# liruihan000/game_engine

Hardware: AMD Instinct MI355X
Metric: room-phase steps/sec (higher is better)
Workload: dtype u32

## Files before the change

game_engine_amd/csrc/ge_device.h:

```cpp
#pragma once
#include <hip/hip_runtime.h>
#include "ge_layout.h"

namespace ge {

enum { COMP_UI = 0, COMP_TIMER = 1, COMP_ACTION = 2 };
enum { ACT_NONE = 0, ACT_WOLF_TARGET, ACT_DOCTOR_PROTECT, ACT_DETECTIVE, ACT_DAY_VOTE,
       ACT_TT_STATEMENTS, ACT_TT_LIE, ACT_TT_VOTE };
enum { EFF_NONE = 0, EFF_ASSIGN_ROLES, EFF_NIGHT_BEGIN, EFF_NIGHT_RESOLVE, EFF_DAY_RESOLVE,
       EFF_TT_ROUND_START, EFF_TT_REVEAL, EFF_TT_SCORE };
enum { RES_ALWAYS = 0, RES_WOLVES_ZERO, RES_WOLVES_GE_VILLAGERS, RES_FOLLOWS_DAY, RES_FOLLOWS_NIGHT,
       RES_ALL_ROUNDS_DONE, RES_OTHERWISE };

constexpr uint32_t GOLDEN = 0x9E3779B9u;

#ifndef GE_SINGLE_GLOBAL
#define GE_SINGLE_GLOBAL 5
#endif
template <bool LOWOCC, bool SINGLE> constexpr bool single_global(int game_bit) { return SINGLE && ((GE_SINGLE_GLOBAL >> (game_bit + (LOWOCC ? 0 : 1))) & 1) != 0; }
#ifndef GE_DEAL_EARLY
#define GE_DEAL_EARLY 1
#endif
#ifndef GE_STAMPS
#define GE_STAMPS 0
#endif
#ifndef GE_RES_PACKED
#define GE_RES_PACKED 1
#endif
#ifndef GE_QUEUE_PRIO
#define GE_QUEUE_PRIO 3
#endif
#ifndef GE_RES_ATOMIC64
#define GE_RES_ATOMIC64 1
#endif
#ifndef GE_RESOLVE_PRIO
#define GE_RESOLVE_PRIO 2
#endif
#ifndef GE_TALLY_BYTES
#define GE_TALLY_BYTES 1
#endif
#ifndef GE_COLD_FALLBACK
#define GE_COLD_FALLBACK 1
#endif
#ifndef GE_COLD_DEAL_NOW
#define GE_COLD_DEAL_NOW 0
#endif
#ifndef GE_LONE_DEAL_WORDS
#define GE_LONE_DEAL_WORDS 1
#endif
#ifndef GE_TAIL_KNOWN_RESTART
#define GE_TAIL_KNOWN_RESTART 1
#endif
#ifndef GE_ROW_DERIVED
#define GE_ROW_DERIVED 1
#endif
#ifndef GE_CTX_PERM
#define GE_CTX_PERM 0
#endif
#ifndef GE_SKIP_MASK
#define GE_SKIP_MASK 0
#endif
#ifndef GE_RES_UNMASKED
#define GE_RES_UNMASKED 0
#endif
#ifndef GE_ROWS_SPLIT
#define GE_ROWS_SPLIT 1
#endif
#ifndef GE_DEAL_PERIOD
#define GE_DEAL_PERIOD 16
#endif

template <int NB, bool LOWOCC, bool SINGLE = false> struct WwBuild {
    static constexpr bool ORD = NB <= 8;
    static constexpr bool ONE_ATOMIC = NB <= 8 && LOWOCC;
    static constexpr bool SHADOW = LOWOCC || NB <= 8;
    static constexpr bool ONEHOT = LOWOCC && NB <= 8;
    static constexpr bool PIN_CHOICE = LOWOCC && NB > 8;
    static constexpr bool SEL_OPEN = LOWOCC;
    static constexpr bool TPL_TRACE = LOWOCC;
    static constexpr int DEAL_FORM = SINGLE ? 2 : NB <= 8 ? ((LOWOCC && !GE_LONE_DEAL_WORDS) ? 0 : 1) : LOWOCC ? 0 : 2;
    static constexpr bool DEAL_EARLY = GE_DEAL_EARLY && !LOWOCC && !SINGLE;
    static constexpr bool TABLE = !LOWOCC;
    static constexpr bool LONE = LOWOCC && NB <= 8 && !SINGLE;
};

GE_HD uint32_t mix32(uint32_t x) {
    x ^= x >> 16; x *= 0x7FEB352Du; x ^= x >> 15; x *= 0x846CA68Bu; x ^= x >> 16;
    return x;
}
GE_HD uint32_t room_key(uint32_t seed_lo, uint32_t seed_hi, uint64_t room) {
    uint32_t k = mix32(seed_lo ^ 0x243F6A88u);
    k = mix32(k ^ seed_hi);
    k = mix32(k ^ (uint32_t)room);
    k = mix32(k ^ (uint32_t)(room >> 32));
    return k;
}
GE_HD uint32_t seed_key(uint32_t seed_lo, uint32_t seed_hi) { return mix32(mix32(seed_lo ^ 0x243F6A88u) ^ seed_hi); }
GE_HD uint32_t room_key_from(uint32_t sk, uint64_t room) { return mix32(mix32(sk ^ (uint32_t)room) ^ (uint32_t)(room >> 32)); }
GE_HD uint32_t turn_key(uint32_t rk, uint32_t turn) { return mix32(rk ^ (turn * GOLDEN)); }
GE_HD uint32_t draw(uint32_t tk, uint32_t idx) { return mix32(tk + (idx + 1u) * GOLDEN); }
GE_HD uint32_t deal_key(uint32_t rk, uint32_t game) { return mix32(rk ^ 0x44454C31u ^ (game * GOLDEN)); }

#if defined(__HIPCC__)
__device__ __forceinline__ uint32_t pick(uint32_t d, uint32_t k) { return __umulhi(d, k); }
__device__ __forceinline__ uint32_t popc(uint32_t x) { return (uint32_t)__popc(x); }
__device__ __forceinline__ uint32_t ctz(uint32_t x) { return (uint32_t)__ffs((int)x) - 1u; }

template <int NB> __device__ __forceinline__ uint32_t nth_set_bit(uint32_t m, uint32_t n) {
    uint32_t pos = 0, c;
    if (NB > 8) { c = popc(m & 0xFFu); if (n >= c) { n -= c; pos = 8; m >>= 8; } }
    c = popc(m & 0xFu); if (n >= c) { n -= c; pos += 4; m >>= 4; }
    c = popc(m & 0x3u); if (n >= c) { n -= c; pos += 2; m >>= 2; }
    c = m & 1u;         if (n >= c) { pos += 1; }
    return pos;
}

__device__ __forceinline__ uint32_t nth_set_bit_swar8(uint32_t m, uint32_t n) {
    uint32_t x = m & 0xFFu;
    x = (x | (x << 12)) & 0x000F000Fu; x = (x | (x << 6)) & 0x03030303u; x = (x | (x << 3)) & 0x11111111u;
    const uint32_t t = (x + 7u - n) * 0x11111111u;
    return (uint32_t)__builtin_ctz((t & 0x88888888u) | 0x80000000u) >> 2;
}

template <int NB> __device__ __forceinline__ uint32_t nth_set_bit_lds(const uint8_t *nth8, uint32_t m, uint32_t n) {
    if (NB <= 8) return nth8[(m & 0xFFu) * 8u + (n & 7u)];
    const uint32_t lo = m & 0xFFu, c = popc(lo);
    const bool in_lo = n < c;
    const uint32_t idx = in_lo ? lo * 8u + n : ((m >> 8) & 0xFFu) * 8u + ((n - c) & 7u);
    return (in_lo ? 0u : 8u) + nth8[idx];
}

inline void fill_nth8_host(uint8_t *nth8) {
    for (uint32_t m = 0; m < 256u; m++) {
        uint32_t x = m;
        for (uint32_t n = 0; n < 8u; n++) {
            uint32_t pos = 0;
            while (x && !((x >> pos) & 1u)) pos++;
            nth8[m * 8u + n] = (uint8_t)(x ? pos : 0u);
            x &= x - 1u;
        }
    }
}

inline void fill_vote_luts_host(uint32_t *spread8, uint64_t *tally64) {
    for (uint32_t m = 0; m < 256u; m++) {
        uint32_t v = 0;
// ... 35 lines not shown
        const uint2 *tally64 = reinterpret_cast<const uint2 *>(static_cast<const unsigned char *>(img) + IMG_TALLY);
        uint32_t v_lo = (uint32_t)votes & spread8[voters & 0xFFu], v_hi = 0;
        if (NB > 8) v_hi = (uint32_t)((uint64_t)votes >> 32) & spread8[(voters >> 8) & 0xFFu];
        uint32_t lo = 0, hi = 0;
#pragma unroll
        for (int k = 0; k < 4; k++) { const uint2 t = tally64[(v_lo >> (8 * k)) & 0xFFu]; lo += t.x; hi += t.y; }
        if (NB > 8) {
#pragma unroll
            for (int k = 0; k < 2; k++) { const uint2 t = tally64[(v_hi >> (8 * k)) & 0xFFu]; lo += t.x; hi += t.y; }
        }
        const uint32_t a = (lo & 0x00F000F0u) | 0x000A000Eu;
        const uint32_t b = ((lo >> 4) & 0x00F000F0u) | 0x0009000Du;
        const uint32_t c = ((lo >> 8) & 0x00F000F0u) | 0x0008000Cu;
        const uint32_t d = ((lo >> 12) & 0x000000F0u) | ((hi & 15u) << 20) | 0x0007000Bu;
        u16x2 m = __builtin_elementwise_max(__builtin_elementwise_max(pk(a), pk(b)), __builtin_elementwise_max(pk(c), pk(d)));
        if (NB > 8) {
            const uint32_t e = (hi & 0x000000F0u) | ((hi << 12) & 0x00F00000u) | 0x00050006u;
            const uint32_t f = ((hi >> 8) & 0x000000F0u) | ((hi << 4) & 0x00F00000u) | 0x00030004u;
            m = __builtin_elementwise_max(m, __builtin_elementwise_max(pk(e), pk(f)));
        }
        const uint32_t key = m.x > m.y ? m.x : m.y;
        return (key >> 4) ? 15u - (key & 15u) : 0u;
    }
    nib_t vm;
    if (NB <= 8) {
        uint32_t x = voters & 0xFFu;
        x = (x | (x << 12)) & 0x000F000Fu; x = (x | (x << 6)) & 0x03030303u; x = (x | (x << 3)) & 0x11111111u;
        vm = (nib_t)nib_fill(x);
    } else {
        uint64_t x = voters & 0xFFFFu;
        x = (x | (x << 24)) & 0x000000FF000000FFull; x = (x | (x << 12)) & 0x000F000F000F000Full;
        x = (x | (x << 6)) & 0x0303030303030303ull; x = (x | (x << 3)) & 0x1111111111111111ull;
        vm = (nib_t)nib_fill(x);
    }
    const nib_t v = votes & vm;
    uint32_t key = 0;
    if (NB <= 8) {
        const uint32_t v32 = (uint32_t)v;
        uint32_t tally = 0;
        if (GE_TALLY_BYTES) {
            const uint32_t ev = (v32 << 2) & 0x3C3C3C3Cu, od = (v32 >> 2) & 0x3C3C3C3Cu, one = 1u;
            tally = (shl_by_byte<0>(one, ev) + shl_by_byte<0>(one, od) + shl_by_byte<1>(one, ev)) + (shl_by_byte<1>(one, od) + shl_by_byte<2>(one, ev))
                  + (shl_by_byte<2>(one, od) + shl_by_byte<3>(one, ev)) + shl_by_byte<3>(one, od);
        } else {
#pragma unroll
            for (int i = 0; i < NB; i++) tally += 1u << ((4u * ((v32 >> (4 * i)) & 15u)) & 31u);
        }
        {
            const uint32_t c8 = popc(v32 & 0x88888888u);
            const uint32_t a = (tally & 0x00F000F0u) | 0x000A000Eu;
            const uint32_t b = ((tally >> 4) & 0x00F000F0u) | 0x0009000Du;
            const uint32_t c = ((tally >> 8) & 0x00F000F0u) | 0x0008000Cu;
            const uint32_t d = ((tally >> 12) & 0x000000F0u) | (c8 << 20) | 0x0007000Bu;
            const u16x2 m = __builtin_elementwise_max(__builtin_elementwise_max(pk(a), pk(b)), __builtin_elementwise_max(pk(c), pk(d)));
            key = m.x > m.y ? m.x : m.y;
        }
    } else {
        uint64_t tally = 0;
#pragma unroll
        for (int i = 0; i < NB; i++) tally += uint64_t(1) << (4u * ((uint32_t)(v >> (4 * i)) & 15u));
        const uint32_t lo = (uint32_t)tally, hi = (uint32_t)(tally >> 32);
        const uint32_t a = (lo & 0x00F000F0u) | 0x000A000Eu;
        const uint32_t b = ((lo >> 4) & 0x00F000F0u) | 0x0009000Du;
        const uint32_t c = ((lo >> 8) & 0x00F000F0u) | 0x0008000Cu;
        const uint32_t d = ((lo >> 12) & 0x000000F0u) | ((hi & 15u) << 20) | 0x0007000Bu;
        const uint32_t e = (hi & 0x000000F0u) | ((hi << 12) & 0x00F00000u) | 0x00050006u;
        const uint32_t f = ((hi >> 8) & 0x000000F0u) | ((hi << 4) & 0x00F00000u) | 0x00030004u;
        const u16x2 m = __builtin_elementwise_max(__builtin_elementwise_max(__builtin_elementwise_max(pk(a), pk(b)), __builtin_elementwise_max(pk(c), pk(d))),
                                                  __builtin_elementwise_max(pk(e), pk(f)));
        key = m.x > m.y ? m.x : m.y;
    }
    return (key >> 4) ? 15u - (key & 15u) : 0u;
}

struct WaveLds {
    uint4 ctx[64];
    uint4 res[64];
    uint8_t queue[64 * 13];
};
struct WaveLdsLow {
    uint4 slot[64 * 13 + 80];
    uint4 res[64];
};
template <bool LOWOCC> struct WaveLdsOf { using type = WaveLds; };
template <> struct WaveLdsOf<true> { using type = WaveLdsLow; };

template <bool SPLIT>
__device__ __forceinline__ DevRow lds_row(const DevRow *rows, uint32_t idx) {
    if (!(SPLIT && GE_ROWS_SPLIT)) return rows[idx];
    const uint4 *h = reinterpret_cast<const uint4 *>(rows);
    const uint4 a = h[idx], b = h[GE_MAX_PHASES + idx];
    return DevRow{a.x, a.y, a.z, a.w, b.x, b.y, b.z, b.w};
}

__device__ __forceinline__ void wave_sync() {
    __builtin_amdgcn_fence(__ATOMIC_RELEASE, "wavefront");
    __builtin_amdgcn_wave_barrier();
    __builtin_amdgcn_fence(__ATOMIC_ACQUIRE, "wavefront");
}

__device__ __forceinline__ void wave_excl_scan(uint32_t cnt, uint32_t &off, uint32_t &total) {
    uint32_t v = cnt;
    v += (uint32_t)__builtin_amdgcn_update_dpp(0, (int)v, 0x111, 0xf, 0xf, false);
    v += (uint32_t)__builtin_amdgcn_update_dpp(0, (int)v, 0x112, 0xf, 0xf, false);
    v += (uint32_t)__builtin_amdgcn_update_dpp(0, (int)v, 0x114, 0xf, 0xf, false);
    v += (uint32_t)__builtin_amdgcn_update_dpp(0, (int)v, 0x118, 0xf, 0xf, false);
    v += (uint32_t)__builtin_amdgcn_update_dpp(0, (int)v, 0x142, 0xa, 0xf, false);
    v += (uint32_t)__builtin_amdgcn_update_dpp(0, (int)v, 0x143, 0xc, 0xf, false);
    off = v - cnt;
    total = (uint32_t)__builtin_amdgcn_readlane((int)v, 63);
}

struct Stamps {
    unsigned long long last, acc[4];
    __device__ __forceinline__ void start() { last = __builtin_amdgcn_s_memtime(); acc[0] = acc[1] = acc[2] = acc[3] = 0; }
    __device__ __forceinline__ void mark(int k) { const unsigned long long now = __builtin_amdgcn_s_memtime(); acc[k] += now - last; last = now; }
    unsigned long long m0, r0;
    __device__ __forceinline__ void clocks_start() { m0 = __builtin_amdgcn_s_memtime(); r0 = __builtin_amdgcn_s_memrealtime(); }
};

__device__ __forceinline__ uint32_t sel32(bool c, uint32_t a, uint32_t b) { return b ^ ((a ^ b) & (0u - (uint32_t)c)); }

template <int NB, bool TABLE>
__device__ __forceinline__ uint32_t ww_choose(uint32_t act, uint32_t i, uint32_t d, uint32_t alive, uint32_t team_w,
                                              uint32_t known, uint32_t lo_kw, uint32_t r_det, const uint8_t *nth8) {
    const uint32_t me = 1u << i;
    const uint32_t others = alive & ~me, non_wolf = alive & ~team_w;
    const uint32_t fresh = others & ~known;
    uint32_t cand;
    if (!TABLE) {
        const uint32_t det_c = sel32(fresh != 0u, fresh, others);
        const uint32_t vote = sel32((team_w & me) != 0u, non_wolf, sel32((r_det & me) != 0u && lo_kw != 0u, lo_kw, others));
        cand = alive;
        cand = sel32(act == ACT_WOLF_TARGET, non_wolf, cand);
        cand = sel32(act == ACT_DETECTIVE, det_c, cand);
        cand = sel32(act == ACT_DAY_VOTE, vote, cand);
        cand = sel32(cand != 0u, cand, alive);
    } else {
        cand = alive;
        cand = act == ACT_WOLF_TARGET ? non_wolf : cand;
        cand = act == ACT_DETECTIVE ? (fresh ? fresh : others) : cand;
        const uint32_t vote = (team_w & me) ? non_wolf : (((r_det & me) && lo_kw) ? lo_kw : others);
        cand = act == ACT_DAY_VOTE ? vote : cand;
        cand = cand ? cand : alive;
    }
    const uint32_t idx = pick(d, popc(cand));
    return (TABLE ? nth_set_bit_lds<NB>(nth8, cand, idx) : NB <= 8 ? nth_set_bit_swar8(cand, idx) : nth_set_bit<NB>(cand, idx)) + 1u;
}

__device__ __forceinline__ uint32_t bit_mask(uint32_t x, uint32_t pos) {
    uint32_t m = (uint32_t)__builtin_amdgcn_sbfe((int)x, pos, 1u);
    asm("" : "+v"(m));
    return m;
}
__device__ __forceinline__ uint32_t bfi(uint32_t m, uint32_t a, uint32_t b) { return (m & a) | (~m & b); }
__device__ __forceinline__ uint32_t bfi_uniform(uint32_t m, uint32_t a, uint32_t b) {
    uint32_t r;
    asm("v_bfi_b32 %0, %1, %2, %3" : "=v"(r) : "v"(m), "s"(a), "v"(b));
    return r;
}

__device__ __forceinline__ uint32_t ww_choose_onehot8(uint32_t x, uint32_t i, uint32_t d, uint32_t known, uint32_t lo_kw, uint32_t det_voter) {
    const uint32_t alive = x & 0xFFFFu, team_w = (x >> 16) & 0xFFFu;
    const uint32_t me = 1u << i;
    const uint32_t others = alive & ~me, non_wolf = alive & ~team_w;
    const uint32_t fresh = others & ~known;
// ... 309 lines not shown
    uint32_t n, nw, phase0_idx, rkey;
    uint32_t human;
    uint32_t term_mask;
};

enum { TAIL_NONE = 0, TAIL_RUNTIME = 1, TAIL_RECYCLE = 2, TAIL_KEEP = 3 };
template <int NB> struct WwRestart {
    const WWR<NB> *s0;
    uint32_t term_rs;
    uint32_t restarted;
    uint32_t q;
};

template <int NB, bool LOWOCC, int GENERIC, bool DER = false>
__device__ __forceinline__ uint32_t ww_targets(const WWR<NB> &s, const DevRow &row, const WwCtx &c, uint32_t alive, uint32_t ALL) {
    using R = WWR<NB>;
    const uint32_t comp = row.r0 & 3u, nterms = (row.r0 >> 8) & 7u;
    uint32_t T = 0;
    const bool generic_row = GENERIC && (row.r0 & ROW_GENERIC);
    if (LOWOCC ? !GENERIC || !generic_row : (comp == COMP_ACTION && !generic_row)) {
        uint32_t X;
        if (NB <= 8) {
            X = __builtin_amdgcn_perm(s.W[1], s.W[0], row.r4) & __builtin_amdgcn_perm(s.W[2], s.W[2], row.r5);
            X ^= row.r7;
            X &= X >> 16; X &= X >> 8;
        } else {
            X = __builtin_amdgcn_perm(s.W[1], s.W[0], row.r4) & __builtin_amdgcn_perm(s.W[R::NW > 3 ? 3 : 0], s.W[2], row.r5) &
                __builtin_amdgcn_perm(s.W[R::NW - 1], s.W[R::NW - 2], row.r6);
            X ^= row.r7;
            X &= X >> 16;
            if (nterms > 2u) {
                auto term = [&](uint32_t j) -> uint32_t {
                    const uint32_t e = (row.r1 >> (8u * j)) & 255u;
                    const uint32_t wi = e >> 5;
                    uint32_t word = 0xFFFFFFFFu;
#pragma unroll
                    for (int k = 0; k < R::NW; k++) word = wi == (uint32_t)k ? s.W[k] : word;
                    const uint32_t m = word >> (e & 31u);
                    return m ^ (uint32_t)((int32_t)(row.r0 << (15u - j)) >> 31);
                };
                X &= term(2) & term(3);
            }
        }
        T = DER ? X & alive & row.r6 : X & alive & (comp == COMP_ACTION ? ALL : 0u);
    }
    if (generic_row && comp == COMP_ACTION)
        T = ww_cond_generic<NB>(s, c.cc, row.r0, ALL) & alive;
    return T;
}

struct WwBranch {
    bool open;
    uint32_t qe;
};
template <int NB>
__device__ __forceinline__ void ww_phase_branch(const WWR<NB> &s, const DevRow &row, uint32_t phase0_idx, uint32_t alive, uint32_t team_w, WwBranch &b) {
    const bool guard = s.phase == phase0_idx && !(s.flags & FLAG_PHASE0_DONE);
    b.open = !guard;
    const uint32_t w = popc(alive & team_w), g = popc(alive & s.template get<F_TEAM_V>());
    static_assert(EFF_DAY_RESOLVE == 4 && RES_FOLLOWS_DAY == 3 && EFF_NIGHT_RESOLVE == 3 && RES_FOLLOWS_NIGHT == 4 && FLAG_PHASE0_DONE == 1,
                  "the constant below is made for these codes");
    const uint32_t follows = (0xC00u >> (s.flags & 0xEu)) & 0x18u;
    const uint32_t C = 1u | ((w == 0u) << RES_WOLVES_ZERO) | ((w >= g) << RES_WOLVES_GE_VILLAGERS) | follows | (1u << RES_OTHERWISE);
    const uint32_t hit = row.r2 & __builtin_amdgcn_perm(C, C, 0u);
    const uint32_t sh = ctz(hit) & 24u;
    b.qe = hit != 0u ? ((row.r3 >> sh) & 255u) : s.phase;
}

template <int NB, bool LOWOCC, bool SINGLE, bool COLD = false>
__device__ __forceinline__ void ww_prepare_deal(const WWR<NB> &s, const WwCtx &c, Deal &deal, bool deal_now, uint32_t ALL, WWR<NB> &dealt) {
    using B = WwBuild<NB, LOWOCC, SINGLE>;
    const uint32_t g = deal_next_game<NB>(s);
    if ((COLD ? __builtin_expect(deal_now, false) : deal_now) && deal.gv != (g | DEAL_VALID)) {
        deal_roles<NB, B::TABLE, B::DEAL_FORM>(deal, deal_key(c.rkey, g), g, c.n, c.nw, c.nth8);
    }
    if (B::DEAL_FORM != DEAL_PACKED) deal_words<NB, B::DEAL_FORM>(deal, ALL, dealt);
}

struct WwActs { uint32_t newly, det_v, det_w; };

template <int NB, bool LOWOCC, bool FUSED = false, bool LONE8 = false, bool SKIP_GIVEN = false, typename S1, typename S2>
__device__ __forceinline__ void ww_queue_actions(WWR<NB> &s, const WwCtx &c, uint32_t T, uint32_t act, bool night, uint32_t alive, uint32_t team_w,
                                                 uint32_t r_det, uint32_t tk, WwActs &out, S1 &&shadow1, S2 &&shadow2, Stamps *stamps,
                                                 uint32_t rowd = 0u, uint32_t nmask = 0u, uint32_t skip = 0u) {
    using nib_t = typename WWR<NB>::nib_t;
    using B = WwBuild<NB, LOWOCC>;
    constexpr bool DER = LONE8 && GE_ROW_DERIVED, PERM = LONE8 && GE_CTX_PERM && NB <= 8, UNMASKED = LONE8 && GE_RES_UNMASKED && B::ONE_ATOMIC;
    constexpr bool SKIPM = GE_SKIP_MASK && SKIP_GIVEN;
    auto *lw = static_cast<typename WaveLdsOf<LOWOCC>::type *>(c.wave_lds);
    const uint32_t todo = SKIPM ? (T & ~s.acted & ~skip) : c.valid ? (T & ~s.acted & ~c.human) : 0u;
    const uint32_t known = s.det_v | s.det_w;
    const uint32_t kw_alive = s.det_w & alive;
    const uint32_t lo_kw = kw_alive & (0u - kw_alive);
    const uint32_t lane = __lane_id();
    const uint32_t cnt = popc(todo);
#if GE_QUEUE_PRIO
    if (!LOWOCC) __builtin_amdgcn_s_setprio(GE_QUEUE_PRIO);
#endif
    uint32_t ord = 0;
    if (B::ORD) ord = c.ord8[todo & 0xFFu];
    uint32_t off, total;
    wave_excl_scan(cnt, off, total);
    out.newly = 0; out.det_v = 0; out.det_w = 0;
    if (!(LOWOCC || total != 0u)) {
#if GE_QUEUE_PRIO
        __builtin_amdgcn_s_setprio(0);
#endif
        shadow1();
        shadow2();
        return;
    }
    const uint32_t ky = DER ? bfi(nmask, known, lo_kw != 0u ? r_det : 0u) : night ? known : (B::ONEHOT ? (lo_kw != 0u ? r_det : 0u) : r_det);
    const uint32_t kind = B::ONEHOT ? ((1u << act) >> 1) : act;
    static_assert(F_ALIVE == 0 && F_TEAM_W == 7, "the selector below is made for this layout");
    const uint32_t at = PERM ? __builtin_amdgcn_perm(s.W[1], s.W[0], 0x0C070C00u) : alive | (team_w << 16);
    const uint32_t x0 = DER ? at | (rowd & (0xFu << ROWD_KIND_SHIFT)) : at | (kind << 28);
    const uint4 ctx = B::ORD ? make_uint4(x0, ky | (lo_kw << 8) | (off << 16) | (lane << 26), ord, tk)
                             : make_uint4(alive | (team_w << 16) | (act << 28), ky | (lo_kw << 16), todo | (off << 16) | (lane << 26), tk);
    constexpr uint32_t RW = (NB <= 8 && GE_RES_PACKED) ? 2u : 4u;
    uint32_t *const res_w = reinterpret_cast<uint32_t *>(lw->res);
    if (NB <= 8) *reinterpret_cast<uint2 *>(res_w + RW * lane) = make_uint2(0u, 0u);
    else lw->res[lane] = make_uint4(0u, 0u, 0u, 0u);
    if (LOWOCC) {
        auto *lo = reinterpret_cast<WaveLdsLow *>(lw);
        uint4 *qp = lo->slot + (cnt != 0u ? off : 64u * 13u + lane);
#pragma unroll
        for (int j = NB - 1; j >= 0; j--) {
            qp[j] = ctx;
            asm volatile("" ::: "memory");
        }
    } else {
        auto *hi = reinterpret_cast<WaveLds *>(lw);
        hi->ctx[lane] = ctx;
        if (cnt != 0u) {
            uint8_t *qp = hi->queue + off;
#pragma unroll
            for (int j = NB - 1; j >= 0; j--) {
                qp[j] = (uint8_t)lane;
                asm volatile("" ::: "memory");
            }
        }
    }
    wave_sync();
    auto fetch = [&](uint32_t k) -> uint4 {
        if (LOWOCC) return reinterpret_cast<WaveLdsLow *>(lw)->slot[k];
        auto *hi = reinterpret_cast<WaveLds *>(lw);
        return hi->ctx[hi->queue[k] & 63u];
    };
    uint4 c4 = fetch(lane);
    if (B::SHADOW) shadow1();
    constexpr bool PEEL = LOWOCC && FUSED && B::SHADOW;
    if (PEEL) {
        auto round = [&](uint32_t base, auto first_c) {
            const uint32_t k = base + lane;
            if (GE_STAMPS == 1 && stamps && base == 0u) { asm volatile("" :: "v"(c4.x)); stamps->mark(1); }
            uint32_t L, i, know, lokw;
            if (B::ORD) {
                L = c4.y >> 26;
                const uint32_t rank = (k - ((c4.y >> 16) & 0x3FFu)) & 7u;
                i = (c4.z >> (4u * rank)) & 7u;
                know = c4.y & 0xFFu; lokw = (c4.y >> 8) & 0xFFu;
            } else {
                L = c4.z >> 26;
                const uint32_t due = c4.z & 0xFFFFu, rank = (k - ((c4.z >> 16) & 0x3FFu)) & 15u;
                i = nth_set_bit<NB>(due | (1u << 31), rank) & 15u;
                know = c4.y & 0xFFFFu; lokw = c4.y >> 16;
            }
            const uint32_t d = draw(c4.w, i);
            const bool go = k < total && (d & 3u) != 0u;
            uint32_t ch = B::ONEHOT ? ww_choose_onehot8(c4.x, i, d, know, lokw, know)
                                    : ww_choose<NB, false>(c4.x >> 28, i, d, c4.x & 0xFFFFu, (c4.x >> 16) & 0xFFFu, know, lokw, know, c.nth8);
            if (B::PIN_CHOICE) asm volatile("" : "+v"(ch));
            if (UNMASKED && decltype(first_c)::value) {
                atomicOr(res_w + RW * L + 1, go ? ch << (4u * i) : 0u);
            } else if (go) {
                uint32_t *r = res_w + RW * L;
                if (!B::ONE_ATOMIC) atomicOr(r, 1u << i);
                atomicOr(r + 1 + (i >> 3), ch << (4u * (i & 7u)));
            }
        };
        shadow2();
        round(0u, std::true_type{});
        for (uint32_t base = 64u; base < total; base += 64u) {
            c4 = fetch(base + lane);
            round(base, std::false_type{});
        }
    } else {
        for (uint32_t base = 0;; base += 64u) {
            const uint32_t k = base + lane;
            if (GE_STAMPS == 1 && stamps && base == 0u) { asm volatile("" :: "v"(c4.x)); stamps->mark(1); }
            uint32_t L, i, know, lokw;
            if (B::ORD) {
                L = c4.y >> 26;
                const uint32_t rank = (k - ((c4.y >> 16) & 0x3FFu)) & 7u;
                i = (c4.z >> (4u * rank)) & 7u;
                know = c4.y & 0xFFu; lokw = (c4.y >> 8) & 0xFFu;
            } else {
                L = c4.z >> 26;
                const uint32_t due = c4.z & 0xFFFFu, rank = (k - ((c4.z >> 16) & 0x3FFu)) & 15u;
                i = (LOWOCC ? nth_set_bit<NB>(due | (1u << 31), rank) : nth_set_bit_lds<NB>(c.nth8, due, rank)) & 15u;
                know = c4.y & 0xFFFFu; lokw = c4.y >> 16;
            }
            const uint32_t d = draw(c4.w, i);
            const bool go = k < total && (d & 3u) != 0u;
            if (LOWOCC) {
                uint32_t ch = B::ONEHOT ? ww_choose_onehot8(c4.x, i, d, know, lokw, know)
                                        : ww_choose<NB, false>(c4.x >> 28, i, d, c4.x & 0xFFFFu, (c4.x >> 16) & 0xFFFu, know, lokw, know, c.nth8);
                if (B::PIN_CHOICE) asm volatile("" : "+v"(ch));
                if (go) {
                    uint32_t *r = res_w + RW * L;
                    if (!B::ONE_ATOMIC) atomicOr(r, 1u << i);
                    atomicOr(r + 1 + (i >> 3), ch << (4u * (i & 7u)));
                }
            } else if (go) {
                const uint32_t ch = ww_choose<NB, true>(c4.x >> 28, i, d, c4.x & 0xFFFFu, (c4.x >> 16) & 0xFFFu, know, lokw, know, c.nth8);
                uint32_t *r = res_w + RW * L;
                if (NB <= 8 && GE_RES_PACKED && GE_RES_ATOMIC64) {
                    atomicOr(reinterpret_cast<unsigned long long *>(r), (unsigned long long)(1u << i) | ((unsigned long long)(ch << (4u * i)) << 32));
                } else {
                    atomicOr(r, 1u << i);
                    atomicOr(r + 1 + (i >> 3), ch << (4u * (i & 7u)));
                }
            }
            if (base + 64u >= total) break;
            c4 = fetch(k + 64u);
        }
    }
    wave_sync();
    const uint4 r = NB <= 8 ? make_uint4(reinterpret_cast<const uint2 *>(res_w + RW * lane)->x, reinterpret_cast<const uint2 *>(res_w + RW * lane)->y, 0u, 0u)
                            : lw->res[lane];
    if (B::SHADOW) {
        if (!PEEL) shadow2();
// ... 92 lines not shown
        if (B::DEAL_FORM == DEAL_PACKED) deal_words<NB, B::DEAL_FORM>(deal, ALL, dealt);
#pragma unroll
        for (int k = 0; k < R::NW; k++) s.W[k] = (s.W[k] & ~dmask.W[k]) | dealt.W[k];
        deal.gv = 0u;
    } else if (eff == EFF_NIGHT_RESOLVE || eff == EFF_DAY_RESOLVE) {
#if GE_RESOLVE_PRIO
        __builtin_amdgcn_s_setprio(GE_RESOLVE_PRIO);
#endif
        resolve(true, eff == EFF_DAY_RESOLVE);
#if GE_RESOLVE_PRIO
        __builtin_amdgcn_s_setprio(0);
#endif
    }
    const bool nbeg = eff == EFF_NIGHT_BEGIN;
    s.template clear<F_SUB>(nbeg ? R::FM : 0u);
    s.sel = nbeg ? nib_t(0) : s.sel;
    if (!TAILR) {
        s.acted = 0; s.choice = 0;
        s.flags = (s.flags & FLAG_PHASE0_DONE) | (p_eff << 1);
        s.prev = s.phase;
        s.phase = q;
        const bool terminal = SINGLE ? ((c.term_mask >> q) & 1u) != 0u : ((qrow.r0 >> 11) & 7u) == 0u;
        s.end_turn = (terminal && s.end_turn == END_NONE) ? (turn < 0xFFFEu ? turn : 0xFFFEu) : s.end_turn;
    } else {
        s.acted &= ~moved; s.choice &= (nib_t)~moved;
        s.flags = bfi(moved, GE_ROW_DERIVED ? (row.r6 >> ROWD_FLAGS_SHIFT) & 0xFFu : (s.flags & FLAG_PHASE0_DONE) | (p_eff << 1), s.flags);
        s.prev = bfi(moved, s.phase, s.prev);
        s.phase = q;
        if (TAILR != TAIL_RECYCLE) {
            const bool terminal = ((qrow.r0 >> 11) & 7u) == 0u;
            s.end_turn = (terminal && moved != 0u && s.end_turn == END_NONE) ? (turn < 0xFFFEu ? turn : 0xFFFEu) : s.end_turn;
        }
    }
    if (TAILR == TAIL_RUNTIME || TAILR == TAIL_RECYCLE) {
#pragma unroll
        for (int k = 0; k < R::NW; k++) s.W[k] = bfi_uniform(rmask, s0->W[k], s.W[k]);
        s.acted |= rmask & s0->acted; s.choice |= (nib_t)rmask & s0->choice;
        s.det_v = bfi_uniform(rmask, s0->det_v, s.det_v); s.det_w = bfi_uniform(rmask, s0->det_w, s.det_w);
        s.sel = (nib_t)bfi_uniform(rmask, (uint32_t)s0->sel, (uint32_t)s.sel);
        s.phase = bfi_uniform(rmask, s0->phase, s.phase); s.prev = bfi_uniform(rmask, s0->prev, s.prev);
        s.flags = bfi_uniform(rmask, s0->flags, s.flags); s.end_turn = bfi_uniform(rmask, s0->end_turn, s.end_turn);
        const uint32_t g = s.games - rmask;
        s.games = g < 0xFFFFu ? g : 0xFFFFu;
    }
}

template <int NB, bool LOWOCC, int GENERIC = false, bool SINGLE = false, int TAILR = TAIL_NONE>
__device__ __forceinline__ void ww_turn(WWR<NB> &s, DevRow &row, const WwCtx &c, uint32_t turn, uint32_t &tk_io, bool trace, Deal &deal, bool deal_now,
                                        uint32_t &ev_newly, uint64_t &ev_choice, Stamps *stamps = nullptr, WwRestart<NB> *rst = nullptr, uint32_t skip = 0u) {
    static_assert(!TAILR || (NB <= 8 && LOWOCC && !SINGLE), "tail recycling is the fused lone-wavefront Werewolf x 8 form");
    using R = WWR<NB>;
    using B = WwBuild<NB, LOWOCC, SINGLE>;
    const uint32_t ALL = (1u << c.n) - 1u;
    const uint32_t comp = row.r0 & 3u, act = (row.r0 >> 2) & 7u;
    const uint32_t alive = s.template get<F_ALIVE>(), team_w = s.template get<F_TEAM_W>(), r_det = s.template get<F_DET>();
    const bool night = act >= ACT_WOLF_TARGET && act <= ACT_DETECTIVE;

    constexpr bool LONE8 = B::LONE && GENERIC == 0, DER = LONE8 && GE_ROW_DERIVED;
    const uint32_t rowd = row.r6, nmask = DER ? bit_mask(rowd, ROWD_NIGHT_BIT) : 0u;

    const uint32_t T = ww_targets<NB, LOWOCC, GENERIC, DER>(s, row, c, alive, ALL);
    if (GE_STAMPS == 1 && stamps) { asm volatile("" :: "v"(T)); stamps->mark(0); }

    WwBranch br;
    R dealt;
    if (B::DEAL_EARLY) ww_prepare_deal<NB, LOWOCC, SINGLE>(s, c, deal, deal_now, ALL, dealt);
    uint32_t tk_next = 0;
    WwActs acts;
    ww_queue_actions<NB, LOWOCC, !SINGLE, LONE8, TAILR == TAIL_RECYCLE || TAILR == TAIL_KEEP>(s, c, T, act, night, alive, team_w, r_det, tk_io, acts,
        [&]() {
            ww_phase_branch<NB>(s, row, c.phase0_idx, alive, team_w, br);
            if (B::SHADOW) asm volatile("" : "+v"(br.qe));
        },
        [&]() {
            if (!SINGLE) tk_next = turn_key(c.rkey, turn + 1u);
            if (!B::DEAL_EARLY) ww_prepare_deal<NB, LOWOCC, SINGLE, TAILR != TAIL_NONE && GE_COLD_DEAL_NOW>(s, c, deal, deal_now, ALL, dealt);
            if (B::SHADOW) {
                if (!SINGLE) asm volatile("" : "+v"(tk_next));
                if (B::DEAL_FORM != DEAL_PACKED && !B::DEAL_EARLY && !(LOWOCC && B::DEAL_FORM == DEAL_WORDS)) {
#pragma unroll
                    for (int k = 0; k < R::NW; k++) asm volatile("" : "+v"(dealt.W[k]));
                }
            }
        }, stamps, rowd, nmask, skip);
    s.acted |= acts.newly;
    s.template set<F_SUB>(DER ? acts.newly & nmask : night ? acts.newly : 0u);
    ev_newly = acts.newly;
    if (trace) {
        uint64_t m = 0;
#pragma unroll
        for (int i = 0; i < NB; i++) m |= (uint64_t)((acts.newly >> i) & 1u) << (4 * i);
        ev_choice = (uint64_t)s.choice & nib_fill(m);
    }

    tk_io = tk_next;
    s.flags |= FLAG_PHASE0_DONE;
    const uint32_t qe = ww_decide<NB, LOWOCC, DER>(s, comp, T, br);
    {
        const uint32_t seen = acts.det_v | acts.det_w;
        s.det_v = (s.det_v & ~seen) | acts.det_v;
        s.det_w = (s.det_w & ~seen) | acts.det_w;
    }
    if (SINGLE) {
        if ((qe & 31u) != s.phase) ww_apply_effect<NB, LOWOCC, true>(s, row, row, c, qe, alive, ALL, turn, deal, dealt);
    } else if (TAILR) {
        const uint32_t q = qe & 31u;
        const uint32_t moved = 0u - (uint32_t)(q != s.phase);
        const uint32_t rmask = TAILR == TAIL_KEEP ? 0u : bit_mask(rst->term_rs, q);
        const DevRow qrow = lds_row<false>(c.rows, TAILR == TAIL_KEEP ? q : bfi_uniform(rmask, c.phase0_idx, q));
        ww_apply_effect<NB, LOWOCC, false, TAILR>(s, row, qrow, c, qe, alive, ALL, turn, deal, dealt, rmask, rst->s0, moved);
        row = qrow;
        rst->q = q;
        rst->restarted = rmask & 1u;
    } else if ((qe & 31u) != s.phase) {
        const DevRow qrow = lds_row<!LOWOCC>(c.rows, qe & 31u);
        ww_apply_effect<NB, LOWOCC, false>(s, row, qrow, c, qe, alive, ALL, turn, deal, dealt);
        row = qrow;
    }
}

template <int NB> __device__ __forceinline__ uint32_t tt_done_mask(uint64_t rounds_nib, uint32_t R) {
    uint32_t m = 0;
#pragma unroll
    for (int i = 0; i < NB; i++) m |= (((uint32_t)(rounds_nib >> (4 * i)) & 15u) >= R ? 1u : 0u) << i;
    return m;
}

template <int NB, bool QUEUE, bool TABLE, int GENERIC = false, bool SINGLE = false>
__device__ __forceinline__ void tt_turn(TT<NB> &s, uint32_t &done, DevRow &row, const DevRow *rows, const CondCtx &cc, void *wave_lds, const uint8_t *nth8,
                                        bool valid, uint32_t n, uint32_t rounds,
                                        uint32_t phase0_idx, uint32_t rkey, uint32_t turn,
                                        bool trace, uint32_t human, uint32_t term_mask, uint32_t &ev_newly, uint64_t &ev_choice) {
    const uint32_t ALL = (1u << n) - 1u;
    const uint32_t comp = row.r0 & 3u, act = (row.r0 >> 2) & 7u, p_eff = (row.r0 >> 5) & 7u;
    const uint32_t nterms = (row.r0 >> 8) & 7u;
    const uint32_t tk = turn_key(rkey, turn);

    uint32_t T = 0;
    const bool generic_row = GENERIC && (row.r0 & ROW_GENERIC);
    if (comp == COMP_ACTION && !generic_row) {
        const uint32_t W0 = s.speaker | (s.submitted << 16), W1 = s.revealed | (s.can_vote << 16), W2 = s.has_voted;
        uint32_t X = __builtin_amdgcn_perm(W1, W0, row.r4) & __builtin_amdgcn_perm(W2, W2, row.r5);
        X ^= row.r7;
        X &= X >> 16;
        if (nterms > 2u) {
            auto term = [&](uint32_t j) -> uint32_t {
                const uint32_t e = (row.r1 >> (8u * j)) & 255u;
                const uint32_t wi = e >> 5;
                uint32_t word = 0xFFFFFFFFu;
                word = wi == 0u ? W0 : word; word = wi == 1u ? W1 : word; word = wi == 2u ? W2 : word;
                const uint32_t m = word >> (e & 31u);
                return m ^ (uint32_t)((int32_t)(row.r0 << (15u - j)) >> 31);
            };
            X &= term(2) & term(3);
        }
        T = X & ALL;
    }
    if (generic_row && comp == COMP_ACTION)
        T = tt_cond_generic<NB, GENERIC>(s, cc, row.r0, ALL);

    uint32_t newly = 0;
    {
        uint32_t todo = valid ? (T & ~s.acted & ~human) : 0u;
        const bool a_stm = act == ACT_TT_STATEMENTS, a_lie = act == ACT_TT_LIE, a_vote = act == ACT_TT_VOTE;
        if (!QUEUE) {
            while (todo) {
                const uint32_t i = ctz(todo);
// ... 127 lines not shown
```

game_engine_amd/csrc/ge_step.hip:

```cpp
#include <hip/hip_runtime.h>
#include <stdint.h>
#include <stdio.h>
#include <stdlib.h>
#include <string.h>
#include <sched.h>
#include <algorithm>
#include <atomic>
#include <new>
#include <string>
#include <thread>
#include <type_traits>
#include <vector>

#include "../../include/ge_step.h"
#include "ge_device.h"
#include "ge_layout.h"
#include "ge_host.h"

using namespace ge;

namespace {

#include "ge_kernels.inl"

// ... 240 lines not shown
                s.dev.base = reinterpret_cast<uint32_t *>(static_cast<char *>(b->state) + reinterpret_cast<size_t>(s.dev.base));
                DevTable &dt = host_tables[k];
                memset(&dt, 0, sizeof dt);
                for (int r = 0; r < s.table.n_phases; r++) {
                    dt.rows[r] = to_dev_row(s.table, s.table.rows[r], s.dev.kind, s.dev.n_players);
                    dt.conds[r] = to_dev_cond(s.table.rows[r]);
                    if (s.table.rows[r].generic) b->generic = true;
                }
                build_cond_image(s.table, s.dev.kind, dt);
                b->cond_bytes = std::max<uint32_t>(b->cond_bytes, dt.cond_n16 * 16u);
                if (b->segs.size() == 1 && s.table.pack == GE_PACK_TWO_TRUTHS && dt.cond_n16) {
                    static const bool no_shapes = getenv("GE_NO_GENERIC_SHAPES") != nullptr;
                    const uint32_t ncl = dt.cond_shape & 7u, len = (dt.cond_shape >> 4) & 7u;
                    b->gshape = no_shapes ? 0u : (ncl == 1u && len == 1u) ? 2u : (ncl == 1u && len == 2u) ? 3u : 0u;
                }
                dt.n_phases = s.table.n_phases; dt.rounds = s.table.rounds; dt.n_players = (int32_t)s.dev.n_players;
                fill_nth8_host(dt.nth8);
                fill_ord8_host(dt.ord8);
                fill_vote_luts_host(dt.spread8, dt.tally64);
                ge_room_view v;
                memset(&v, 0, sizeof v);
                v.phase_id = 0; v.prev_phase_id = 0; v.end_turn = -1; v.n_players = (uint8_t)s.dev.n_players;
                v.pack = (uint8_t)s.table.pack;
                for (uint32_t i = 0; i < s.dev.n_players; i++) memcpy(v.players[i], s.table.init_fields, 12);
                uint32_t w[12] = {0};
                view_to_words(s.dev.kind, v, s.table, w);
                memcpy(s.dev.init_words, w, sizeof w);
                init_regs_of(s.dev.kind, w, s.dev.init_regs);
                s.dev.done0 = 0;
                if (s.table.pack == GE_PACK_TWO_TRUTHS)
                    for (uint32_t i = 0; i < s.dev.n_players; i++)
                        if ((int)(v.players[i][8] & 15) >= s.table.rounds) s.dev.done0 |= 1u << i;
                for (int r = 0; r < s.table.n_phases; r++)
                    if (s.table.rows[r].n_branches == 0) s.dev.term_mask |= 1u << r;
            }
            if (hipMemcpy(b->tables, host_tables.data(), sizeof(DevTable) * host_tables.size(), hipMemcpyHostToDevice) != hipSuccess) { st = GE_ERR_HIP; break; }
            std::vector<int32_t> ids(b->segs.size() * GE_MAX_PHASES, 0);
            for (size_t k = 0; k < b->segs.size(); k++)
                for (int r = 0; r < b->segs[k].table.n_phases; r++) ids[k * GE_MAX_PHASES + r] = b->segs[k].table.rows[r].phase_id;
            if (hipMalloc(reinterpret_cast<void **>(&b->phase_ids), sizeof(int32_t) * ids.size()) != hipSuccess ||
                hipMemcpy(b->phase_ids, ids.data(), sizeof(int32_t) * ids.size(), hipMemcpyHostToDevice) != hipSuccess) { st = GE_ERR_HIP; break; }
            SegDev host[GE_MAX_SEGMENTS];
            memset(host, 0, sizeof host);
            for (size_t k = 0; k < b->segs.size(); k++) host[k] = b->segs[k].dev;
            if (hipMemcpy(b->segs_dev, host, sizeof host, hipMemcpyHostToDevice) != hipSuccess) { st = GE_ERR_HIP; break; }
        } while (0);
    }
    if (st != GE_OK) { ge_batch_destroy(b); return st; }
#if GE_STAMPS
    if (getenv("GE_STAMPS_OUT")) {
        DeviceGuard dg(b->device);
        const size_t sb = 64 + (GE_STAMPS == 2 ? 32 * (size_t)((b->n_rooms + 63) / 64 + 64) : 0);
        if (hipMalloc(reinterpret_cast<void **>(&b->stamps_dev), sb) == hipSuccess) (void)hipMemset(b->stamps_dev, 0, sb);
    }
#endif
    st = ge_batch_reset(b);
    if (st != GE_OK) { ge_batch_destroy(b); return st; }
    *out = b;
    return GE_OK;
}

static int sync_impl(ge_batch *b) {
    HIP_TRY(hipStreamSynchronize(b->last_stream));
    b->pending = false;
    return GE_OK;
}

static int reset_impl(ge_batch *b) {
    GE_ON_DEVICE(b);
    int st = sync_impl(b);
    if (st != GE_OK) return st;
    b->turn = 0;
    uint64_t most = 0;
    for (const Segment &s : b->segs) most = s.dev.rooms_padded > most ? s.dev.rooms_padded : most;
    const uint32_t blocks = (uint32_t)((most / 256u) < 2048u ? (most / 256u) : 2048u);
    hipLaunchKernelGGL(ge_fill_kernel, dim3(blocks ? blocks : 1u), dim3(256), 0, b->last_stream, b->segs_dev, (uint32_t)b->segs.size());
    HIP_TRY(hipGetLastError());
    return sync_impl(b);
}

namespace {
struct LaunchShape { dim3 grid, block; hipStream_t st; const ge_batch *b; StepArgs a; };

template <class K> inline void launch_one(K kernel, const LaunchShape &L, bool queue, bool lds_low) {
    StepArgs a = L.a;
    const uint32_t base = step_lds_bytes(queue, lds_low, L.block.x);
    a.cond_off = base;
    hipLaunchKernelGGL(kernel, L.grid, L.block, base + (L.b->generic ? L.b->cond_bytes : 0u), L.st, L.b->segs_dev, L.b->tables, a);
}

template <bool LOW, int GEN, bool SINGLE> inline void launch_kind(uint32_t kind, const LaunchShape &L) {
    constexpr bool HAS_ALT = SINGLE && !LOW && GEN == 0;
    constexpr bool NO_RECYCLE = GE_TAIL_KNOWN_RESTART && LOW && !SINGLE && GEN == 0;
    const bool alt = HAS_ALT && L.b->stream_loads != (kind != K_WW8);
    switch (kind) {
    case K_WW8:
        if (alt) launch_one(ge_step_kernel<K_WW8, LOW, GEN, SINGLE, HAS_ALT ? 2 : 0>, L, true, LOW);
        else if (NO_RECYCLE && !L.a.restart) launch_one(ge_step_kernel<K_WW8, LOW, GEN, SINGLE, NO_RECYCLE ? LD_NO_RECYCLE : 0>, L, true, LOW);
        else launch_one(ge_step_kernel<K_WW8, LOW, GEN, SINGLE>, L, true, LOW);
        break;
    case K_WW12:
        if (alt) launch_one(ge_step_kernel<K_WW12, LOW, GEN, SINGLE, HAS_ALT ? 1 : 0>, L, true, LOW);
        else launch_one(ge_step_kernel<K_WW12, LOW, GEN, SINGLE>, L, true, LOW);
        break;
    case K_TT4:
        if (alt) launch_one(ge_step_kernel<K_TT4, LOW, GEN, SINGLE, HAS_ALT ? 1 : 0>, L, tt_uses_queue(4, LOW), LOW);
        else launch_one(ge_step_kernel<K_TT4, LOW, GEN, SINGLE>, L, tt_uses_queue(4, LOW), LOW);
        break;
    case K_TT8:
        if (alt) launch_one(ge_step_kernel<K_TT8, LOW, GEN, SINGLE, HAS_ALT ? 1 : 0>, L, tt_uses_queue(8, LOW), LOW);
        else launch_one(ge_step_kernel<K_TT8, LOW, GEN, SINGLE>, L, tt_uses_queue(8, LOW), LOW);
        break;
    default:
        if (alt) launch_one(ge_step_kernel<K_TT12, LOW, GEN, SINGLE, HAS_ALT ? 1 : 0>, L, tt_uses_queue(12, LOW), LOW);
        else launch_one(ge_step_kernel<K_TT12, LOW, GEN, SINGLE>, L, tt_uses_queue(12, LOW), LOW);
        break;
    }
}
template <bool LOW, int GEN> inline void launch_kind(uint32_t kind, bool single, const LaunchShape &L) {
    if (single) launch_kind<LOW, GEN, true>(kind, L); else launch_kind<LOW, GEN, false>(kind, L);
}
template <bool LOW, int GEN> inline void launch_tt_shaped(uint32_t kind, const LaunchShape &L) {
    switch (kind) {
    case K_TT4: launch_one(ge_step_kernel<K_TT4, LOW, GEN, false>, L, tt_uses_queue(4, LOW), LOW); break;
    case K_TT8: launch_one(ge_step_kernel<K_TT8, LOW, GEN, false>, L, tt_uses_queue(8, LOW), LOW); break;
    default: launch_one(ge_step_kernel<K_TT12, LOW, GEN, false>, L, tt_uses_queue(12, LOW), LOW); break;
    }
}
template <bool LOW> inline void launch_tt_shaped(uint32_t gshape, uint32_t kind, const LaunchShape &L) {
    if (gshape == 2u) launch_tt_shaped<LOW, 2>(kind, L); else launch_tt_shaped<LOW, 3>(kind, L);
}
template <bool LOW, int GEN> inline void launch_mixed(bool single, const LaunchShape &L) {
    if (single) launch_one(ge_step_kernel_mixed<LOW, GEN, true>, L, true, LOW); else launch_one(ge_step_kernel_mixed<LOW, GEN, false>, L, true, LOW);
}
}

static void launch_geometry(const ge_batch *b, bool low, bool single, uint32_t &bt, uint32_t &blocks, uint32_t &rpb) {
    bt = b->block_threads; blocks = b->n_blocks;
    rpb = bt;
    static const uint32_t single_block_env = [] {
        const char *e = getenv("GE_SINGLE_BLOCK");
        const unsigned long v = e ? strtoul(e, nullptr, 10) : 0ul;
        return (v == 256 || v == 512 || v == 1024) ? (uint32_t)v : 0u;
    }();
    if (single && b->segs.size() == 1 && !b->generic && !low && bt == 256u) {
        bt = single_block_env ? single_block_env : (b->segs[0].dev.kind == K_WW8 && b->segs[0].dev.rooms >= 393216u ? 512u : 256u);
        blocks = (uint32_t)((b->segs[0].dev.rooms + bt - 1u) / bt);
        rpb = bt;
    }
    if (single && b->segs.size() == 1 && !low && bt < 256u && single_block_env == 0u) {
        bt = 256u;
        blocks = (uint32_t)((b->segs[0].dev.rooms + bt - 1u) / bt);
        rpb = bt;
    }
    static const int half_env = [] { const char *e = getenv("GE_HALF_WAVES"); return e ? atoi(e) : -1; }();
    const bool half_fits = b->segs.size() == 1 && low && bt == 64u && (!single || half_env == 1);
    if (half_fits && (half_env == 1 || (half_env != 0 && b->segs[0].dev.rooms <= 32768u))) {
        rpb = 32u;
        blocks = (uint32_t)((b->segs[0].dev.rooms + 31u) / 32u);
    } else if (half_fits && half_env != 0 && b->segs[0].dev.rooms < 65536u) {
        rpb = (uint32_t)((b->segs[0].dev.rooms + 1023u) / 1024u);
        blocks = (uint32_t)((b->segs[0].dev.rooms + rpb - 1u) / rpb);
    }
}

static bool launch_low(const ge_batch *b, const StepArgs &a) {
    return a.lowocc != 0u && !(b->generic && b->segs.size() > 1);
}

static hipError_t launch_step(const ge_batch *b, const StepArgs &a_in, hipStream_t st) {
    const bool single = a_in.n_turns == 1u, mixed = b->segs.size() > 1, low = launch_low(b, a_in);
    uint32_t bt, blocks, rpb;
    launch_geometry(b, low, single, bt, blocks, rpb);
    LaunchShape L{dim3(blocks), dim3(bt), st, b, a_in};
    L.a.block_threads = bt;
    L.a.rooms_per_block = rpb;
    const uint32_t kind = b->segs[0].dev.kind;
    if (mixed) {
        if (b->generic) launch_mixed<false, 1>(single, L);
        else if (low) launch_mixed<true, 0>(single, L);
        else launch_mixed<false, 0>(single, L);
    } else if (b->generic) {
// ... 539 lines not shown
```

Baseline: 73.90 billion.

## Replace per-slot context copies with pull-style queue for lone 8-player wavefronts

```diff
diff --git a/game_engine_amd/csrc/ge_device.h b/game_engine_amd/csrc/ge_device.h
--- a/game_engine_amd/csrc/ge_device.h
+++ b/game_engine_amd/csrc/ge_device.h
@@ -62,6 +62,9 @@
 #endif
 #ifndef GE_RES_UNMASKED
 #define GE_RES_UNMASKED 0
+#endif
+#ifndef GE_PULL_QUEUE
+#define GE_PULL_QUEUE 1
 #endif
 #ifndef GE_ROWS_SPLIT
 #define GE_ROWS_SPLIT 1
@@ -263,6 +266,12 @@
     uint4 slot[64 * 13 + 80];
     uint4 res[64];
 };
+struct WaveLdsPull {
+    uint4 cctx[128];
+    uint4 res[64];
+    uint32_t head[64 * 13];
+};
+static_assert(sizeof(WaveLdsPull) <= sizeof(WaveLdsLow) && sizeof(WaveLdsPull) % 16 == 0, "the pull form lives in a lone wavefront's queue memory");
 template <bool LOWOCC> struct WaveLdsOf { using type = WaveLds; };
 template <> struct WaveLdsOf<true> { using type = WaveLdsLow; };
 
@@ -738,9 +747,11 @@
 template <int NB, bool LOWOCC, bool FUSED = false, bool LONE8 = false, bool SKIP_GIVEN = false, typename S1, typename S2>
 __device__ __forceinline__ void ww_queue_actions(WWR<NB> &s, const WwCtx &c, uint32_t T, uint32_t act, bool night, uint32_t alive, uint32_t team_w,
                                                  uint32_t r_det, uint32_t tk, WwActs &out, S1 &&shadow1, S2 &&shadow2, Stamps *stamps,
-                                                 uint32_t rowd = 0u, uint32_t nmask = 0u, uint32_t skip = 0u) {
+                                                 uint32_t rowd = 0u, uint32_t nmask = 0u, uint32_t skip = 0u, uint32_t qstamp = 0u) {
     using nib_t = typename WWR<NB>::nib_t;
     using B = WwBuild<NB, LOWOCC>;
+    constexpr int PULL = LONE8 ? GE_PULL_QUEUE : 0;
+    auto *pq = static_cast<WaveLdsPull *>(c.wave_lds);
     constexpr bool DER = LONE8 && GE_ROW_DERIVED, PERM = LONE8 && GE_CTX_PERM && NB <= 8, UNMASKED = LONE8 && GE_RES_UNMASKED && B::ONE_ATOMIC;
     constexpr bool SKIPM = GE_SKIP_MASK && SKIP_GIVEN;
     auto *lw = static_cast<typename WaveLdsOf<LOWOCC>::type *>(c.wave_lds);
@@ -774,10 +785,23 @@
     const uint4 ctx = B::ORD ? make_uint4(x0, ky | (lo_kw << 8) | (off << 16) | (lane << 26), ord, tk)
                              : make_uint4(alive | (team_w << 16) | (act << 28), ky | (lo_kw << 16), todo | (off << 16) | (lane << 26), tk);
     constexpr uint32_t RW = (NB <= 8 && GE_RES_PACKED) ? 2u : 4u;
-    uint32_t *const res_w = reinterpret_cast<uint32_t *>(lw->res);
+    uint32_t *const res_w = PULL ? reinterpret_cast<uint32_t *>(pq->res) : reinterpret_cast<uint32_t *>(lw->res);
     if (NB <= 8) *reinterpret_cast<uint2 *>(res_w + RW * lane) = make_uint2(0u, 0u);
     else lw->res[lane] = make_uint4(0u, 0u, 0u, 0u);
-    if (LOWOCC) {
+    if (PULL == 1) {
+        const uint64_t nz = __builtin_amdgcn_ballot_w64(cnt != 0u);
+        const uint32_t r = __builtin_amdgcn_mbcnt_hi((uint32_t)(nz >> 32), __builtin_amdgcn_mbcnt_lo((uint32_t)nz, 0u));
+        pq->cctx[cnt != 0u ? r : 64u + lane] = ctx;
+        pq->head[off] = qstamp;
+    } else if (PULL == 2) {
+        pq->cctx[lane] = ctx;
+        uint8_t *qp = reinterpret_cast<uint8_t *>(pq->head) + (cnt != 0u ? off : 64u * 13u + lane);
+#pragma unroll
+        for (int j = NB - 1; j >= 0; j--) {
+            qp[j] = (uint8_t)lane;
+            asm volatile("" ::: "memory");
+        }
+    } else if (LOWOCC) {
         auto *lo = reinterpret_cast<WaveLdsLow *>(lw);
         uint4 *qp = lo->slot + (cnt != 0u ? off : 64u * 13u + lane);
 #pragma unroll
@@ -798,12 +822,21 @@
         }
     }
     wave_sync();
-    auto fetch = [&](uint32_t k) -> uint4 {
+    uint32_t heads_before = 0;
+    auto fetch = [&](uint32_t k, bool first = false) -> uint4 {
+        if (PULL == 1) {
+            const bool is_head = pq->head[k] == qstamp;
+            const uint64_t hb = __builtin_amdgcn_ballot_w64(is_head), above = hb >> 1;
+            const uint32_t at0 = first ? 0u : heads_before + ((uint32_t)hb & 1u) - 1u;
+            heads_before += (uint32_t)__builtin_popcountll(hb);
+            return pq->cctx[__builtin_amdgcn_mbcnt_hi((uint32_t)(above >> 32), __builtin_amdgcn_mbcnt_lo((uint32_t)above, at0))];
+        }
+        if (PULL == 2) return pq->cctx[reinterpret_cast<const uint8_t *>(pq->head)[k] & 63u];
         if (LOWOCC) return reinterpret_cast<WaveLdsLow *>(lw)->slot[k];
         auto *hi = reinterpret_cast<WaveLds *>(lw);
         return hi->ctx[hi->queue[k] & 63u];
     };
-    uint4 c4 = fetch(lane);
+    uint4 c4 = fetch(lane, true);
     if (B::SHADOW) shadow1();
     constexpr bool PEEL = LOWOCC && FUSED && B::SHADOW;
     if (PEEL) {
@@ -1062,7 +1095,11 @@
                     for (int k = 0; k < R::NW; k++) asm volatile("" : "+v"(dealt.W[k]));
                 }
             }
+#if GE_PULL_QUEUE == 1
+        }, stamps, rowd, nmask, skip, turn + 1u);
+#else
         }, stamps, rowd, nmask, skip);
+#endif
     s.acted |= acts.newly;
     s.template set<F_SUB>(DER ? acts.newly & nmask : night ? acts.newly : 0u);
     ev_newly = acts.newly;
diff --git a/game_engine_amd/csrc/ge_step.hip b/game_engine_amd/csrc/ge_step.hip
--- a/game_engine_amd/csrc/ge_step.hip
+++ b/game_engine_amd/csrc/ge_step.hip
@@ -346,9 +346,9 @@
 namespace {
 struct LaunchShape { dim3 grid, block; hipStream_t st; const ge_batch *b; StepArgs a; };
 
-template <class K> inline void launch_one(K kernel, const LaunchShape &L, bool queue, bool lds_low) {
+template <class K> inline void launch_one(K kernel, const LaunchShape &L, bool queue, bool lds_low, bool lds_pull = false) {
     StepArgs a = L.a;
-    const uint32_t base = step_lds_bytes(queue, lds_low, L.block.x);
+    const uint32_t base = step_lds_bytes(queue, lds_low, L.block.x, lds_pull);
     a.cond_off = base;
     hipLaunchKernelGGL(kernel, L.grid, L.block, base + (L.b->generic ? L.b->cond_bytes : 0u), L.st, L.b->segs_dev, L.b->tables, a);
 }
@@ -360,8 +360,8 @@
     switch (kind) {
     case K_WW8:
         if (alt) launch_one(ge_step_kernel<K_WW8, LOW, GEN, SINGLE, HAS_ALT ? 2 : 0>, L, true, LOW);
-        else if (NO_RECYCLE && !L.a.restart) launch_one(ge_step_kernel<K_WW8, LOW, GEN, SINGLE, NO_RECYCLE ? LD_NO_RECYCLE : 0>, L, true, LOW);
-        else launch_one(ge_step_kernel<K_WW8, LOW, GEN, SINGLE>, L, true, LOW);
+        else if (NO_RECYCLE && !L.a.restart) launch_one(ge_step_kernel<K_WW8, LOW, GEN, SINGLE, NO_RECYCLE ? LD_NO_RECYCLE : 0>, L, true, LOW, pull_queue_kernel(K_WW8, LOW, GEN, SINGLE));
+        else launch_one(ge_step_kernel<K_WW8, LOW, GEN, SINGLE>, L, true, LOW, pull_queue_kernel(K_WW8, LOW, GEN, SINGLE));
         break;
     case K_WW12:
         if (alt) launch_one(ge_step_kernel<K_WW12, LOW, GEN, SINGLE, HAS_ALT ? 1 : 0>, L, true, LOW);
```

New measurement: 76.88 billion (median of 6 runs). 1.04x the previous value.
